# guohaoqiang/Flex

Measured on AMD Instinct MI355X. Metric: SpMM GFLOPS (2*nnz*k/t), higher is better.
Workload: dtype f32

## Files before the change

### flex_amd/csrc/spmm_bf16_kernels.hip

```cpp
#include <cstdint>

#include "attention_device.h"
#include "plan.h"
#include "spmm_device.h"

namespace flex {
namespace spmm_bf16 {

using namespace spmm_dev;
using attention::bf16_bits;

struct Acc8 {
    float4 lo, hi;
};

__device__ __forceinline__ void fma8(Acc8 &acc, float v, const float4 &w) {
    const uint32_t w0 = __float_as_uint(w.x), w1 = __float_as_uint(w.y), w2 = __float_as_uint(w.z), w3 = __float_as_uint(w.w);
    acc.lo.x = fmaf(v, as_f32(w0 << 16), acc.lo.x);
    acc.lo.y = fmaf(v, as_f32(w0 & 0xFFFF0000u), acc.lo.y);
    acc.lo.z = fmaf(v, as_f32(w1 << 16), acc.lo.z);
    acc.lo.w = fmaf(v, as_f32(w1 & 0xFFFF0000u), acc.lo.w);
    acc.hi.x = fmaf(v, as_f32(w2 << 16), acc.hi.x);
    acc.hi.y = fmaf(v, as_f32(w2 & 0xFFFF0000u), acc.hi.y);
    acc.hi.z = fmaf(v, as_f32(w3 << 16), acc.hi.z);
    acc.hi.w = fmaf(v, as_f32(w3 & 0xFFFF0000u), acc.hi.w);
}

__device__ __forceinline__ v4u narrow8(const float4 &lo, const float4 &hi) {
    const v4u r = {bf16_bits(lo.x) | (bf16_bits(lo.y) << 16), bf16_bits(lo.z) | (bf16_bits(lo.w) << 16),
                   bf16_bits(hi.x) | (bf16_bits(hi.y) << 16), bf16_bits(hi.z) | (bf16_bits(hi.w) << 16)};
    return r;
}

template <int G, bool OFF32, int U>
__device__ __forceinline__ void compute_chunk_bf16(const PlanView &p, const ChunkRegs &d, uint2 *my_lds, const char *__restrict__ Bb,
                                                   uint32_t *__restrict__ Cw, int lane, int c0, bool col_ok, uint32_t tile) {
    constexpr int S = 64 / G;
    const int slot = lane / G;
    const uint64_t ldc = static_cast<uint64_t>(p.ldc);
    const uint32_t lane_off = (col_ok ? c0 : c0 - (lane % G) * 4) * 4u;
    const uint64_t row_bytes = static_cast<uint64_t>(p.ldb) * 4u;
    const uint4 hdr = d.hdr;
    const uint2 cx = d.cx;
    const uint32_t my_beg = d.my_beg, my_dst = d.my_dst;

    const uint32_t nt = hdr.y, zb = hdr.z, ze = hdr.w;
    const bool packed_chunk = p.rec_packed != 0 && (cx.y & kChunkWide) == 0;
    const uint2 *__restrict__ rec = p.rec_packed != 0 ? p.rec + cx.x - zb : p.rec;
    uint32_t carry = 0;

    uint32_t ti = 0;
    uint32_t row_end = __builtin_amdgcn_readlane(my_beg, 1);
    Acc8 acc = {{0.f, 0.f, 0.f, 0.f}, {0.f, 0.f, 0.f, 0.f}};
    const bool out_ok = col_ok && slot == 0;
    auto flush = [&](uint32_t pos) {
        do {
            const uint32_t dst = __builtin_amdgcn_readlane(my_dst, ti);
            if ((dst & (kPartialFlag | kBundleFlag)) == (kPartialFlag | kBundleFlag)) {
                if constexpr (kTileHasBundles<G>) {
                    const uint32_t first = dst & (kBundleRowsPerChunk - 1u);
                    const uint32_t held = first < 64u ? d.my_bd0 : d.my_bd1;
                    const uint32_t row = static_cast<uint32_t>(
                        __builtin_amdgcn_ds_bpermute(static_cast<int>(((first & 63u) + slot) << 2), static_cast<int>(held)));
                    if (col_ok && row != kBundleNoRow) {
                        const bool none = (row & kBundleZero) != 0;
                        const v4u zero = {0u, 0u, 0u, 0u};
                        const v4u val = none ? zero : narrow8(acc.lo, acc.hi);
                        __builtin_nontemporal_store(val, reinterpret_cast<v4u *>(Cw + static_cast<uint64_t>(row & ~kBundleZero) * ldc + c0));
                    }
                }
            } else if (__builtin_expect((dst & kPartialFlag) != 0, 0)) {
                const float4 lo = reduce_full<G>(acc.lo), hi = reduce_full<G>(acc.hi);
                if (out_ok) {
                    int l = lane;
                    asm volatile("" : "+v"(l));
                    const int col = 2 * (static_cast<int>(tile) * (4 * G) + (l % G) * 4);
                    float *prow = p.partial + static_cast<uint64_t>(dst & ~kPartialFlag) * (2u * static_cast<uint32_t>(p.k)) + col;
                    *reinterpret_cast<float4 *>(prow) = lo;
                    *reinterpret_cast<float4 *>(prow + 4) = hi;
                }
            } else {
                const float4 lo = reduce_full<G>(acc.lo), hi = reduce_full<G>(acc.hi);
                if (out_ok) __builtin_nontemporal_store(narrow8(lo, hi), reinterpret_cast<v4u *>(Cw + static_cast<uint64_t>(dst) * ldc + c0));
            }
            acc = {{0.f, 0.f, 0.f, 0.f}, {0.f, 0.f, 0.f, 0.f}};
            ++ti;
            row_end = ti < nt ? __builtin_amdgcn_readlane(my_beg, ti + 1) : 0xFFFFFFFFu;
        } while (row_end == pos);
    };
    if (nt == 0) row_end = 0xFFFFFFFFu;
    if (row_end == zb) flush(zb);

    uint32_t pos = zb;
    for (uint32_t wz = zb; wz < ze; wz += kWindowRecs<G>) {
        const uint32_t wn = min(static_cast<uint32_t>(kWindowRecs<G>), ze - wz);
        if (packed_chunk) carry = stage_window_packed<G, OFF32>(p, my_lds, zb, wz, wn, cx, hdr.x, nt, my_beg, carry, static_cast<uint32_t>(row_bytes), lane);
        else stage_window<G>(my_lds, rec, wz, wn, lane, p.rec_nt != 0);
        const uint32_t nsteps = wn / S;
        const uint2 *lds_slot = my_lds + slot;
        uint32_t j = 0;
        for (; j + U <= nsteps; j += U) {
            uint2 r[U];
            float4 b[U];
#pragma unroll
            for (int u = 0; u < U; ++u) r[u] = lds_slot[(j + u) * S];
#pragma unroll
            for (int u = 0; u < U; ++u) b[u] = gather4<OFF32>(Bb, r[u].x, lane_off, row_bytes);
#pragma unroll
            for (int u = 0; u < U; ++u) {
                fma8(acc, as_f32(r[u].y), b[u]);
                pos += S;
                if (pos == row_end) flush(pos);
            }
        }
        if (j < nsteps) {
            uint2 r[U];
            float4 b[U];
#pragma unroll
            for (int u = 0; u < U; ++u) r[u] = lds_slot[min(j + u, nsteps - 1) * S];
#pragma unroll
            for (int u = 0; u < U; ++u) b[u] = gather4<OFF32>(Bb, r[u].x, lane_off, row_bytes);
#pragma unroll
            for (int u = 0; u < U; ++u) {
                if (j + u < nsteps) {
                    fma8(acc, as_f32(r[u].y), b[u]);
                    pos += S;
                    if (pos == row_end) flush(pos);
                }
            }
        }
    }
}

template <int G, bool OFF32>
constexpr int kWavesHint = G == 64 && OFF32 ? 6 : G >= 32 ? 5 : 7;

template <int G, bool OFF32, int U, int WPB>
__global__ __launch_bounds__(64 * WPB) __attribute__((amdgpu_waves_per_eu(kWavesHint<G, OFF32>))) void spmm_flat_bf16_kernel(PlanView p, const flex_bf16 *__restrict__ B,
                                                                                                                  flex_bf16 *__restrict__ C) {
    __shared__ uint2 lds_rec[WPB][kWindowRecs<G>];
    const int lane = threadIdx.x & 63;
    const uint32_t wib = __builtin_amdgcn_readfirstlane(threadIdx.x >> 6);
    uint32_t tile, ktiles, chunk;
    if (!place_of_wave<G, WPB>(p, wib, tile, ktiles, chunk)) return;
    const int c0 = tile * (4 * G) + (lane % G) * 4;
    const bool col_ok = c0 < p.k;
    ChunkRegs d;
    if (!load_chunk<G>(p, chunk, lane, d)) return;
    compute_chunk_bf16<G, OFF32, U>(p, d, lds_rec[wib], reinterpret_cast<const char *>(B), reinterpret_cast<uint32_t *>(C), lane, c0, col_ok, tile);
}

__global__ __launch_bounds__(256) void spmm_fixup_bf16_kernel(const float *__restrict__ partial, const SplitRow *__restrict__ rows, uint32_t n_rows,
                                                              int k, int ldcw, uint32_t *__restrict__ Cw) {
    const int lane = threadIdx.x & 63;
    const uint32_t wib = __builtin_amdgcn_readfirstlane(threadIdx.x >> 6);
    const uint32_t i = blockIdx.x * kWavesPerBlock + wib;
    if (i >= n_rows) return;
    const SplitRow sr = rows[i];
    for (int c = lane; c < k / 2; c += 64) {
        const float *p = partial + static_cast<uint64_t>(sr.first) * k + 2 * c;
        float2 s = make_float2(0.f, 0.f);
        uint32_t j = 0;
        for (; j + 8 <= sr.count; j += 8) {
            float2 v[8];
#pragma unroll
            for (int u = 0; u < 8; ++u) v[u] = *reinterpret_cast<const float2 *>(p + static_cast<uint64_t>(j + u) * k);
#pragma unroll
            for (int u = 0; u < 8; ++u) {
                s.x += v[u].x;
                s.y += v[u].y;
            }
        }
        float2 v[8];
#pragma unroll
        for (int u = 0; u < 8; ++u) v[u] = (j + u < sr.count) ? *reinterpret_cast<const float2 *>(p + static_cast<uint64_t>(j + u) * k) : make_float2(0.f, 0.f);
#pragma unroll
        for (int u = 0; u < 8; ++u)
            if (j + u < sr.count) {
                s.x += v[u].x;
                s.y += v[u].y;
            }
        Cw[static_cast<uint64_t>(sr.row) * ldcw + c] = bf16_bits(s.x) | (bf16_bits(s.y) << 16);
    }
}

template <int G, bool OFF32, int U>
int launch_flat(const PlanView &v, const flex_bf16 *dB, flex_bf16 *dC, hipStream_t s) {
    uint32_t nblk = (v.n_chunks + kWavesPerBlock - 1) / kWavesPerBlock;
    nblk = (nblk + kXcds - 1) / kXcds * kXcds;
    const uint32_t ktiles = (v.k + 4 * G - 1) / (4 * G);
    const dim3 grid = v.tile_group ? dim3(nblk * ktiles, 1) : dim3(nblk, ktiles);
    hipLaunchKernelGGL((spmm_flat_bf16_kernel<G, OFF32, U, kWavesPerBlock>), grid, dim3(64 * kWavesPerBlock), v.lds_extra, s, v, dB, dC);
    FLEX_HIP_TRY(hipGetLastError());
    return FLEX_OK;
}

template <int G, int U>
int launch_flat_off(const PlanView &v, bool off32, const flex_bf16 *dB, flex_bf16 *dC, hipStream_t s) {
    return off32 ? launch_flat<G, true, U>(v, dB, dC, s) : launch_flat<G, false, U>(v, dB, dC, s);
}

int launch(const PlanView &v, int lanes_per_nz, bool off32, const flex_bf16 *dB, flex_bf16 *dC, hipStream_t s) {
    if (v.n_chunks == 0) return FLEX_OK;
    switch (lanes_per_nz) {
        case 4: return launch_flat_off<4, 4>(v, off32, dB, dC, s);
        case 8: return launch_flat_off<8, 4>(v, off32, dB, dC, s);
        case 16: return launch_flat_off<16, 4>(v, off32, dB, dC, s);
        case 32: return launch_flat_off<32, 8>(v, off32, dB, dC, s);
        case 64: return launch_flat_off<64, 8>(v, off32, dB, dC, s);
        default: return FLEX_ERR_UNSUPPORTED;
    }
}

int launch_fixup(const flex_plan *p, flex_bf16 *dC, hipStream_t s) {
    if (p->n_split == 0) return FLEX_OK;
    const uint32_t nblk = (p->n_split + kWavesPerBlock - 1) / kWavesPerBlock;
    hipLaunchKernelGGL(spmm_fixup_bf16_kernel, dim3(nblk), dim3(256), 0, s, p->d_partial.get(), p->d_split.get(), p->n_split, 2 * p->k, p->ldc,
                       reinterpret_cast<uint32_t *>(dC));
    FLEX_HIP_TRY(hipGetLastError());
    return FLEX_OK;
}

}
}

using namespace flex;

extern "C" int flex_spmm_bf16(flex_plan *p, const flex_bf16 *dB, flex_bf16 *dC, flex_stream_t stream) {
    if (!p || !p->bf16) return FLEX_ERR_INVALID;
    if (p->m == 0) return FLEX_OK;
    if (!dC || (!dB && p->nnz > 0)) return FLEX_ERR_INVALID;
    if ((reinterpret_cast<uintptr_t>(dB) | reinterpret_cast<uintptr_t>(dC)) % 16 != 0) return FLEX_ERR_UNSUPPORTED;
    const DeviceScope on(p->device);
    FLEX_HIP_TRY(on.error());
    hipStream_t s = reinterpret_cast<hipStream_t>(stream);
    const LaunchGuard guard(p, s);
    if (guard.begin() != FLEX_OK) return FLEX_ERR_INVALID;
    int rc = spmm_bf16::launch(plan_view(p, false, nullptr), p->lanes_per_nz, p->off32, dB, dC, s);
    if (rc == FLEX_OK) rc = spmm_bf16::launch_fixup(p, dC, s);
    if (rc == FLEX_OK) guard.done();
    return rc;
}
```

### flex_amd/csrc/spmm_device.h

```cpp
#pragma once
#include "internal.h"

namespace flex {
namespace spmm_dev {
__device__ __forceinline__ float as_f32(uint32_t u) { return __uint_as_float(u); }

template <bool OFF32>
__device__ __forceinline__ float4 gather4(const char *__restrict__ Bb, uint32_t recx, uint32_t lane_off,
                                          uint64_t row_bytes) {
    if constexpr (OFF32) {
        return *reinterpret_cast<const float4 *>(Bb + static_cast<uint32_t>(recx + lane_off));
    } else {
        return *reinterpret_cast<const float4 *>(Bb + (static_cast<uint64_t>(recx) * row_bytes + lane_off));
    }
}

__device__ __forceinline__ void fma4(float4 &acc, float v, const float4 &b) {
    acc.x = fmaf(v, b.x, acc.x);
    acc.y = fmaf(v, b.y, acc.y);
    acc.z = fmaf(v, b.z, acc.z);
    acc.w = fmaf(v, b.w, acc.w);
}

typedef float v4f __attribute__((ext_vector_type(4)));
typedef uint32_t v4u __attribute__((ext_vector_type(4)));

__device__ __forceinline__ float pair8(float a, float b) {
    float r;
    asm("s_nop 1\n\t"
        "v_add_f32_dpp %0, %1, %1 row_ror:8 row_mask:0xf bank_mask:0x3\n\t"
        "v_add_f32_dpp %0, %2, %2 row_ror:8 row_mask:0xf bank_mask:0xc"
        : "=&v"(r)
        : "v"(a), "v"(b));
    return r;
}

__device__ __forceinline__ float pair4(float a, float b) {
    float r;
    asm("s_nop 1\n\t"
        "v_add_f32_dpp %0, %1, %1 row_ror:12 row_mask:0xf bank_mask:0x5\n\t"
        "v_add_f32_dpp %0, %2, %2 row_ror:4 row_mask:0xf bank_mask:0xa"
        : "=&v"(r)
        : "v"(a), "v"(b));
    return r;
}

__device__ __forceinline__ float pair16(float a, float b) {
    const auto sw = __builtin_amdgcn_permlane16_swap(__float_as_uint(a), __float_as_uint(b), false, false);
    return __uint_as_float(sw[0]) + __uint_as_float(sw[1]);
}

__device__ __forceinline__ float pair32(float a, float b) {
    const auto sw = __builtin_amdgcn_permlane32_swap(__float_as_uint(a), __float_as_uint(b), false, false);
    return __uint_as_float(sw[0]) + __uint_as_float(sw[1]);
}

template <int G>
__device__ __forceinline__ float4 reduce_full(const float4 &acc) {
    float4 r = acc;
    if constexpr (G <= 4) {
        auto partner = [](float x) {
            const int lo = __builtin_amdgcn_update_dpp(0, __builtin_bit_cast(int, x), 0x12C, 0xf, 0x5, false);
            return __builtin_bit_cast(float, __builtin_amdgcn_update_dpp(lo, __builtin_bit_cast(int, x), 0x124, 0xf, 0xa, false));
        };
        r.x += partner(r.x);
        r.y += partner(r.y);
        r.z += partner(r.z);
        r.w += partner(r.w);
    }
    if constexpr (G <= 8) {
        r.x += __builtin_bit_cast(float, __builtin_amdgcn_update_dpp(0, __builtin_bit_cast(int, r.x), 0x128, 0xf, 0xf, false));
        r.y += __builtin_bit_cast(float, __builtin_amdgcn_update_dpp(0, __builtin_bit_cast(int, r.y), 0x128, 0xf, 0xf, false));
        r.z += __builtin_bit_cast(float, __builtin_amdgcn_update_dpp(0, __builtin_bit_cast(int, r.z), 0x128, 0xf, 0xf, false));
        r.w += __builtin_bit_cast(float, __builtin_amdgcn_update_dpp(0, __builtin_bit_cast(int, r.w), 0x128, 0xf, 0xf, false));
    }
    if constexpr (G <= 16) {
        r.x = pair16(r.x, r.x);
        r.y = pair16(r.y, r.y);
        r.z = pair16(r.z, r.z);
        r.w = pair16(r.w, r.w);
    }
    if constexpr (G <= 32) {
        r.x = pair32(r.x, r.x);
        r.y = pair32(r.y, r.y);
        r.z = pair32(r.z, r.z);
        r.w = pair32(r.w, r.w);
    }
    return r;
}

template <int G>
constexpr int kWindowRecs = G <= 8 ? 512 : 256;
template <int G>
constexpr bool kTileHasBundles = 64 / G >= static_cast<int>(kBundleMinSlots);


typedef uint32_t v2u __attribute__((ext_vector_type(2)));
template <bool NT>
__device__ __forceinline__ uint2 load_rec(const uint2 *ptr) {
    if constexpr (NT) {
        const v2u v = __builtin_nontemporal_load(reinterpret_cast<const v2u *>(ptr));
        return make_uint2(v.x, v.y);
    } else {
        return *ptr;
    }
}

template <bool NT, int LOADS>
__device__ __forceinline__ void stage_n(uint2 *my_lds, const uint2 *__restrict__ rec, uint32_t wz, uint32_t wn, int lane) {
    uint2 r[LOADS];
#pragma unroll
    for (int i = 0; i < LOADS; ++i) r[i] = load_rec<NT>(rec + wz + min(static_cast<uint32_t>(i * 64 + lane), wn - 1));
#pragma unroll
    for (int i = 0; i < LOADS; ++i) my_lds[i * 64 + lane] = r[i];
}

template <bool NT, int G>
__device__ __forceinline__ void stage_window_t(uint2 *my_lds, const uint2 *__restrict__ rec, uint32_t wz, uint32_t wn, int lane) {
    if (wn <= 64) {
        stage_n<NT, 1>(my_lds, rec, wz, wn, lane);
    } else if constexpr (kWindowRecs<G> > 256) {
        if (wn <= 256) stage_n<NT, 4>(my_lds, rec, wz, wn, lane);
        else stage_n<NT, kWindowRecs<G> / 64>(my_lds, rec, wz, wn, lane);
    } else {
        stage_n<NT, 4>(my_lds, rec, wz, wn, lane);
    }
}

template <int G>
__device__ __forceinline__ void stage_window(uint2 *my_lds, const uint2 *__restrict__ rec, uint32_t wz, uint32_t wn, int lane, bool nt) {
    if (nt) stage_window_t<true, G>(my_lds, rec, wz, wn, lane);
    else stage_window_t<false, G>(my_lds, rec, wz, wn, lane);
}

template <bool NT, class T>
__device__ __forceinline__ T load_stream(const T *ptr) {
    if constexpr (NT) return __builtin_nontemporal_load(ptr);
    else return *ptr;
}

template <bool NT, bool PAIR, int LOADS, int R>
__device__ __forceinline__ void stage_packed_n(uint2 *my_lds, const float *__restrict__ val, const uint16_t *__restrict__ dcol, uint32_t wn, int lane,
                                               uint32_t (&vv)[R]) {
    const char *const vb = reinterpret_cast<const char *>(val), *const db = reinterpret_cast<const char *>(dcol);
#pragma unroll
    for (int i = 0; i < R; ++i) vv[i] = 0u;
    if constexpr (PAIR) {
        uint32_t d[LOADS];
#pragma unroll
        for (int i = 0; i < LOADS; ++i) {
            const uint32_t off = min(static_cast<uint32_t>(i * 64 + lane), wn / 2 - 1) * 4u;
            const v2u v = load_stream<NT>(reinterpret_cast<const v2u *>(vb + static_cast<uint32_t>(off * 2u)));
            vv[2 * i] = v.x;
            vv[2 * i + 1] = v.y;
            d[i] = load_stream<NT>(reinterpret_cast<const uint32_t *>(db + off));
        }
#pragma unroll
        for (int i = 0; i < LOADS; ++i) *reinterpret_cast<uint4 *>(my_lds + 2 * (i * 64 + lane)) = make_uint4(d[i] & 0xFFFFu, 0u, d[i] >> 16, 0u);
    } else {
        uint16_t d[LOADS];
#pragma unroll
        for (int i = 0; i < LOADS; ++i) {
            const uint32_t off = min(static_cast<uint32_t>(i * 64 + lane), wn - 1) * 2u;
            vv[i] = __float_as_uint(load_stream<NT>(reinterpret_cast<const float *>(vb + static_cast<uint32_t>(off * 2u))));
            d[i] = load_stream<NT>(reinterpret_cast<const uint16_t *>(db + off));
        }
#pragma unroll
        for (int i = 0; i < LOADS; ++i) my_lds[i * 64 + lane] = make_uint2(d[i], 0u);
    }
}

template <bool NT, int G, int R>
__device__ __forceinline__ void stage_packed_t(uint2 *my_lds, const float *__restrict__ val, const uint16_t *__restrict__ dcol, uint32_t wn, int lane,
                                               uint32_t (&vv)[R]) {
    constexpr bool PAIR = 64 / G >= 2;
    constexpr int PER = PAIR ? 128 : 64, FULL = kWindowRecs<G> / PER;
    if (wn <= PER) stage_packed_n<NT, PAIR, 1>(my_lds, val, dcol, wn, lane, vv);
    else if (FULL > 2 && wn <= 2 * PER) stage_packed_n<NT, PAIR, 2>(my_lds, val, dcol, wn, lane, vv);
    else stage_packed_n<NT, PAIR, FULL>(my_lds, val, dcol, wn, lane, vv);
}

template <int G, bool OFF32>
__device__ __forceinline__ uint32_t stage_window_packed(const PlanView &p, uint2 *my_lds, uint32_t zb, uint32_t wz, uint32_t wn, uint2 cx,
                                                        uint32_t t0, uint32_t nt, uint32_t my_beg, uint32_t carry, uint32_t row_bytes32, int lane) {
    constexpr int W = kWindowRecs<G>, R = W / 64;
    constexpr bool PAIR = 64 / G >= 2;
    asm volatile("" : "+v"(lane));
    uint32_t vv[R];
    if (p.rec_nt != 0) stage_packed_t<true, G>(my_lds, p.rec_val + wz, p.rec_dcol + wz, wn, lane, vv);
    else stage_packed_t<false, G>(my_lds, p.rec_val + wz, p.rec_dcol + wz, wn, lane, vv);
    for (uint32_t j = lane; j < cx.y; j += 64) {
        const uint2 e = p.exc[cx.x + j];
        const uint32_t at = zb + e.x - wz;
        if (at < wn) my_lds[at].x += e.y;
    }
    if (lane == 0) my_lds[0].x += carry;
    const uint32_t next_beg = __shfl_down(my_beg, 1);
    const uint32_t at = my_beg - wz;
    if (static_cast<uint32_t>(lane) < nt && next_beg != my_beg && at < wn) my_lds[at] = make_uint2(p.t_col0[t0 + lane], 1u);
    __builtin_amdgcn_wave_barrier();
    uint32_t w[R], fbits = 0;
#pragma unroll
    for (int i = 0; i < R; ++i) {
        const uint2 s = my_lds[lane * R + i];
        w[i] = s.x;
        fbits |= s.y << i;
    }
    fbits &= (1u << R) - 1u;
    __builtin_amdgcn_wave_barrier();
#pragma unroll
    for (int i = 0; i < R; ++i) my_lds[PAIR ? 2 * ((i / 2) * 64 + lane) + (i & 1) : i * 64 + lane].y = vv[i];
    uint32_t run = 0;
#pragma unroll
    for (int i = 0; i < R; ++i) {
        run = ((fbits >> i) & 1u) ? w[i] : run + w[i];
        w[i] = run;
    }
    uint32_t inc = run;
#pragma unroll
    for (int dlt = 1; dlt < 64; dlt <<= 1) {
        const uint32_t up = __shfl_up(inc, dlt);
        if (lane >= dlt) inc += up;
    }
    const uint32_t exc_sum = inc - run;
    const uint64_t below = __builtin_amdgcn_ballot_w64(fbits != 0) & ((uint64_t(1) << lane) - 1u);
    const int q = below ? 63 - __builtin_clzll(below) : 0;
    const uint32_t e_q = __shfl(exc_sum, q);
    const uint32_t enter = below ? exc_sum - e_q : exc_sum;
    uint32_t last = 0;
#pragma unroll
    for (int i = 0; i < R; ++i) {
        const bool open = (fbits & ((2u << i) - 1u)) == 0;
        const uint32_t col = w[i] + (open ? enter : 0u);
        my_lds[lane * R + i].x = OFF32 ? col * row_bytes32 : col;
        last = col;
    }
    __builtin_amdgcn_wave_barrier();
    return __builtin_amdgcn_readlane(last, 63);
}

template <int G, int WPB>
__device__ __forceinline__ bool place_of_wave(const PlanView &p, uint32_t wib, uint32_t &tile, uint32_t &ktiles, uint32_t &chunk) {
    uint32_t bid;
    tile = blockIdx.y;
    ktiles = gridDim.y;
    if (p.tile_group == 0) {
        const uint32_t cpx = gridDim.x / kXcds;
        bid = p.xcd_remap ? (blockIdx.x % kXcds) * cpx + (blockIdx.x / kXcds) : blockIdx.x;
    } else {
        ktiles = (p.k + 4 * G - 1) / (4 * G);
        const uint32_t nwg = gridDim.x / ktiles;
        const uint32_t slice = p.xcd_remap ? nwg / kXcds : nwg;
        const uint32_t l = p.xcd_remap ? blockIdx.x / kXcds : blockIdx.x;
        const uint32_t g = l / (p.tile_group * ktiles), r = l % (p.tile_group * ktiles);
        const uint32_t g0 = g * p.tile_group, gs = min(p.tile_group, slice - g0);
        tile = r / gs;
        const uint32_t in_slice = g0 + r % gs;
        if (tile >= ktiles) return false;
        bid = p.xcd_remap ? (blockIdx.x % kXcds) * slice + in_slice : in_slice;
    }
    chunk = bid * WPB + wib;
    return chunk < p.n_chunks;
}

struct ChunkRegs {
    uint4 hdr;
    uint2 cx;
    uint32_t my_beg, my_dst;
    uint2 my_aux;
    uint32_t my_bd0, my_bd1;
};

template <int G>
__device__ __forceinline__ bool load_chunk(const PlanView &p, uint32_t chunk, int lane, ChunkRegs &d) {
    const uint4 hdr = d.hdr = p.chunk[chunk];
    uint2 cb = make_uint2(0u, 0u);
    if constexpr (kTileHasBundles<G>)
        if (p.bd_rows != nullptr) cb = p.chunk_bd[chunk];
    uint2 cx = make_uint2(0u, 0u);
    if (p.rec_packed != 0) cx = p.chunk_exc[chunk];
    d.cx = cx;
    if (hdr.y == 0) return false;
    d.my_beg = (static_cast<uint32_t>(lane) <= hdr.y) ? p.t_beg[hdr.x + lane] : 0u;
    d.my_dst = (static_cast<uint32_t>(lane) < hdr.y) ? p.t_dst[hdr.x + lane] : 0u;
    d.my_aux = (static_cast<uint32_t>(lane) < hdr.y) ? p.t_aux[hdr.x + lane] : make_uint2(0u, 0u);
    d.my_bd0 = d.my_bd1 = kBundleNoRow;
    if (kTileHasBundles<G> && cb.y != 0) {
        if (static_cast<uint32_t>(lane) < cb.y) d.my_bd0 = p.bd_rows[cb.x + lane];
        if (static_cast<uint32_t>(lane) + 64u < cb.y) d.my_bd1 = p.bd_rows[cb.x + 64u + lane];
    }
    return true;
}

}
}
```

### flex_amd/csrc/spmm_kernels.hip

```cpp
#include "spmm_device.h"

namespace flex {
namespace {

using namespace spmm_dev;

template <int G>
struct RowOut {
    static constexpr int kVals = G <= 8 ? 1 : 4;
    float v[kVals];
};

template <int G>
__device__ __forceinline__ int row_out_col(int lane, int c0) {
    if constexpr (G == 8) return c0 + 2 * ((lane >> 3) & 1) + ((lane >> 4) & 1);
    else if constexpr (G == 4) return c0 + 2 * ((lane >> 2) & 1) + ((lane >> 3) & 1);
    else return c0;
}

template <int G>
__device__ __forceinline__ bool row_out_lane(int lane) {
    return G == 8 ? lane < 32 : G == 4 ? lane < 16 : lane < G;
}

template <int G>
__device__ __forceinline__ RowOut<G> reduce_row(const float4 &acc) {
    RowOut<G> o;
    if constexpr (G == 8) {
        const float t = pair16(pair8(acc.x, acc.z), pair8(acc.y, acc.w));
        o.v[0] = pair32(t, t);
    } else if constexpr (G == 4) {
        const float t = pair8(pair4(acc.x, acc.z), pair4(acc.y, acc.w));
        const float h = pair16(t, t);
        o.v[0] = pair32(h, h);
    } else {
        float4 r = acc;
        if constexpr (G <= 16) {
            r.x = pair16(r.x, r.x);
            r.y = pair16(r.y, r.y);
            r.z = pair16(r.z, r.z);
            r.w = pair16(r.w, r.w);
        }
        if constexpr (G <= 32) {
            r.x = pair32(r.x, r.x);
            r.y = pair32(r.y, r.y);
            r.z = pair32(r.z, r.z);
            r.w = pair32(r.w, r.w);
        }
        o.v[0] = r.x; o.v[1] = r.y; o.v[2] = r.z; o.v[3] = r.w;
    }
    return o;
}

template <int G>
__device__ __forceinline__ void store_row_out(float *ptr, const RowOut<G> &o) {
    if constexpr (RowOut<G>::kVals == 4) {
        const v4f val = {o.v[0], o.v[1], o.v[2], o.v[3]};
        __builtin_nontemporal_store(val, reinterpret_cast<v4f *>(ptr));
    } else {
        __builtin_nontemporal_store(o.v[0], ptr);
    }
}

__device__ __forceinline__ v4f load_b128_sc1(const float *ptr) {
    v4f v;
    asm volatile("global_load_dwordx4 %0, %1, off sc1" : "=v"(v) : "v"(ptr) : "memory");
    return v;
}

template <int N>
__device__ __forceinline__ void wait_loads(v4f (&v)[N]) {
    static_assert(N == 8, "one batch of the piece sum");
    asm volatile("s_waitcnt vmcnt(0)"
                 : "+v"(v[0]), "+v"(v[1]), "+v"(v[2]), "+v"(v[3]), "+v"(v[4]), "+v"(v[5]), "+v"(v[6]), "+v"(v[7])
                 :
                 : "memory");
}

[[maybe_unused]] __device__ __forceinline__ uint32_t xcc_id() {
    uint32_t x;
    asm volatile("s_getreg_b32 %0, hwreg(HW_REG_XCC_ID)" : "=s"(x));
    return x & (kXcds - 1);
}


template <int G, bool OFF32, int U>
__device__ __forceinline__ void compute_chunk(const PlanView &p, uint4 hdr, uint32_t my_beg, uint32_t my_dst, uint2 my_aux,
                                              uint32_t my_bd0, uint32_t my_bd1, uint2 cx, uint2 *my_lds, const char *__restrict__ Bb,
                                              float *__restrict__ C, int lane, int c0, bool col_ok, uint32_t tile, uint32_t ktiles) {
    constexpr int S = 64 / G;
    const int slot = lane / G;
    const int k = p.k;
    const uint64_t ldc = static_cast<uint64_t>(p.ldc);
    const uint32_t lane_off = (col_ok ? c0 : c0 - (lane % G) * 4) * 4u;
    const uint64_t row_bytes = static_cast<uint64_t>(p.ldb) * 4u;

    const uint32_t nt = hdr.y, zb = hdr.z, ze = hdr.w;
    const bool packed_chunk = p.rec_packed != 0 && (cx.y & kChunkWide) == 0;
    const uint2 *__restrict__ rec = p.rec_packed != 0 ? p.rec + cx.x - zb : p.rec;
    uint32_t carry = 0;

    uint32_t ti = 0;
    uint32_t row_end = __builtin_amdgcn_readlane(my_beg, 1);
    float4 acc = {0.f, 0.f, 0.f, 0.f};
    const int out_col = row_out_col<G>(lane, c0);
    const bool out_ok = col_ok && row_out_lane<G>(lane);
    auto flush = [&](uint32_t pos) {
        do {
            const uint32_t dst = __builtin_amdgcn_readlane(my_dst, ti);
            if ((dst & (kPartialFlag | kBundleFlag)) == (kPartialFlag | kBundleFlag)) {
                if constexpr (kTileHasBundles<G>) {
                    const uint32_t first = dst & (kBundleRowsPerChunk - 1u);
                    const uint32_t held = first < 64u ? my_bd0 : my_bd1;
                    const uint32_t row = static_cast<uint32_t>(
                        __builtin_amdgcn_ds_bpermute(static_cast<int>(((first & 63u) + slot) << 2), static_cast<int>(held)));
                    if (col_ok && row != kBundleNoRow) {
                        const bool none = (row & kBundleZero) != 0;
                        const v4f val = {none ? 0.f : acc.x, none ? 0.f : acc.y, none ? 0.f : acc.z, none ? 0.f : acc.w};
                        __builtin_nontemporal_store(val, reinterpret_cast<v4f *>(C + static_cast<uint64_t>(row & ~kBundleZero) * ldc + c0));
                    }
                }
            } else if (__builtin_expect((dst & kPartialFlag) != 0, 0)) {
                const float4 r = reduce_full<G>(acc);
                float *prow = p.partial + static_cast<uint64_t>(dst & ~kPartialFlag) * k;
                if (slot == 0 && col_ok) {
                    int l = lane;
                    asm volatile("" : "+v"(l));
                    const int col = static_cast<int>(tile) * (4 * G) + (l % G) * 4;
                    if (p.fused_fixup) {
                        const auto prsrc = __builtin_amdgcn_make_buffer_rsrc(prow, 0, k * 4, 0x00020000);
                        const v4u pv = {__float_as_uint(r.x), __float_as_uint(r.y), __float_as_uint(r.z), __float_as_uint(r.w)};
                        __builtin_amdgcn_raw_buffer_store_b128(pv, prsrc, col * 4, 0, 16 );
                    } else {
                        *reinterpret_cast<float4 *>(prow + col) = r;
                    }
                }
            } else {
                const RowOut<G> o = reduce_row<G>(acc);
                if (out_ok) store_row_out<G>(C + static_cast<uint64_t>(dst) * ldc + out_col, o);
            }
            acc = {0.f, 0.f, 0.f, 0.f};
            ++ti;
            row_end = ti < nt ? __builtin_amdgcn_readlane(my_beg, ti + 1) : 0xFFFFFFFFu;
        } while (row_end == pos);
    };
    if (nt == 0) row_end = 0xFFFFFFFFu;
    if (row_end == zb) flush(zb);

    uint32_t pos = zb;
    for (uint32_t wz = zb; wz < ze; wz += kWindowRecs<G>) {
        const uint32_t wn = min(static_cast<uint32_t>(kWindowRecs<G>), ze - wz);
        if (packed_chunk) carry = stage_window_packed<G, OFF32>(p, my_lds, zb, wz, wn, cx, hdr.x, nt, my_beg, carry, static_cast<uint32_t>(row_bytes), lane);
        else stage_window<G>(my_lds, rec, wz, wn, lane, p.rec_nt != 0);
        const uint32_t nsteps = wn / S;
        const uint2 *lds_slot = my_lds + slot;
        uint32_t j = 0;
        for (; j + U <= nsteps; j += U) {
            uint2 r[U];
            float4 b[U];
#pragma unroll
            for (int u = 0; u < U; ++u) r[u] = lds_slot[(j + u) * S];
#pragma unroll
            for (int u = 0; u < U; ++u) b[u] = gather4<OFF32>(Bb, r[u].x, lane_off, row_bytes);
#pragma unroll
            for (int u = 0; u < U; ++u) {
                fma4(acc, as_f32(r[u].y), b[u]);
                pos += S;
                if (pos == row_end) flush(pos);
            }
        }
        if (j < nsteps) {
            uint2 r[U];
            float4 b[U];
#pragma unroll
            for (int u = 0; u < U; ++u) r[u] = lds_slot[min(j + u, nsteps - 1) * S];
#pragma unroll
            for (int u = 0; u < U; ++u) b[u] = gather4<OFF32>(Bb, r[u].x, lane_off, row_bytes);
#pragma unroll
            for (int u = 0; u < U; ++u) {
                if (j + u < nsteps) {
                    fma4(acc, as_f32(r[u].y), b[u]);
                    pos += S;
                    if (pos == row_end) flush(pos);
                }
            }
        }
    }
    const bool mine_partial = static_cast<uint32_t>(lane) < nt && (my_dst & (kPartialFlag | kBundleFlag)) == kPartialFlag;
    if (p.fused_fixup && __builtin_amdgcn_ballot_w64(mine_partial) != 0) {
        asm volatile("s_waitcnt vmcnt(0)" ::: "memory");
        uint32_t arrived = 0;
        if (mine_partial)
            arrived = __hip_atomic_fetch_add(p.split_cnt + static_cast<uint64_t>(my_aux.x) * ktiles + tile, 1u,
                                             __ATOMIC_RELAXED, __HIP_MEMORY_SCOPE_AGENT);
        uint64_t done = __builtin_amdgcn_ballot_w64(mine_partial && arrived + 1 == my_aux.y);
        while (done != 0) {
            int take = -1;
#pragma unroll
            for (int s2 = 0; s2 < S; ++s2) {
                if (done != 0) {
                    const int i = __builtin_ctzll(done);
                    done &= done - 1;
                    if (slot == s2) take = i;
                }
            }
            const uint32_t sidx = __shfl(my_aux.x, take < 0 ? 0 : take);
            if (take >= 0) {
                const SplitRow sr = p.split[sidx];
                if (col_ok) {
                    int l = lane;
                    asm volatile("" : "+v"(l));
                    const int c0 = static_cast<int>(tile) * (4 * G) + (l % G) * 4;
                    const float *base = p.partial + static_cast<uint64_t>(sr.first) * k + c0;
                    float4 s4 = {0.f, 0.f, 0.f, 0.f};
                    for (uint32_t j = 0; j < sr.count; j += 8) {
                        v4f v[8];
#pragma unroll
                        for (int u = 0; u < 8; ++u) v[u] = load_b128_sc1(base + static_cast<uint64_t>(min(j + u, sr.count - 1)) * k);
                        wait_loads(v);
#pragma unroll
                        for (int u = 0; u < 8; ++u) {
                            if (j + u < sr.count) {
                                s4.x += v[u].x;
                                s4.y += v[u].y;
                                s4.z += v[u].z;
                                s4.w += v[u].w;
                            }
                        }
                    }
                    const v4f val = {s4.x, s4.y, s4.z, s4.w};
                    __builtin_nontemporal_store(val, reinterpret_cast<v4f *>(C + static_cast<uint64_t>(sr.row) * ldc + c0));
                }
                if (lane % G == 0)
                    __hip_atomic_store(p.split_cnt + static_cast<uint64_t>(sidx) * ktiles + tile, 0u, __ATOMIC_RELAXED,
                                       __HIP_MEMORY_SCOPE_AGENT);
            }
        }
    }
}

template <int G, bool OFF32, int U, int WPB, bool STAMP = false>
__global__ __launch_bounds__(64 * WPB) __attribute__((amdgpu_waves_per_eu(U == (G >= 32 ? 8 : 4) ? (G >= 32 ? (OFF32 ? 7 : 6) : G >= 16 ? 7 : 8) : 4))) void spmm_flat_kernel(PlanView p, const float *__restrict__ B,
                                                             float *__restrict__ C) {
    __shared__ uint2 lds_rec[WPB][kWindowRecs<G>];
    const int lane = threadIdx.x & 63;
    const uint32_t wib = __builtin_amdgcn_readfirstlane(threadIdx.x >> 6);
    uint32_t tile = blockIdx.y, ktiles = gridDim.y, bid;
    if (p.tile_group == 0) {
        const uint32_t cpx = gridDim.x / kXcds;
        bid = p.xcd_remap ? (blockIdx.x % kXcds) * cpx + (blockIdx.x / kXcds) : blockIdx.x;
    } else {
        ktiles = (p.k + 4 * G - 1) / (4 * G);
        const uint32_t nwg = gridDim.x / ktiles;
        const uint32_t slice = p.xcd_remap ? nwg / kXcds : nwg;
        const uint32_t l = p.xcd_remap ? blockIdx.x / kXcds : blockIdx.x;
        const uint32_t g = l / (p.tile_group * ktiles), r = l % (p.tile_group * ktiles);
        const uint32_t g0 = g * p.tile_group, gs = min(p.tile_group, slice - g0);
        tile = r / gs;
        const uint32_t in_slice = g0 + r % gs;
        if (tile >= ktiles) return;
        bid = p.xcd_remap ? (blockIdx.x % kXcds) * slice + in_slice : in_slice;
    }
    const uint32_t chunk = bid * WPB + wib;
    if (chunk >= p.n_chunks) return;
    const int c0 = tile * (4 * G) + (lane % G) * 4;
    const bool col_ok = c0 < p.k;
    const uint4 hdr = p.chunk[chunk];
    uint2 cb = make_uint2(0u, 0u);
    if constexpr (kTileHasBundles<G>)
        if (p.bd_rows != nullptr) cb = p.chunk_bd[chunk];
    uint2 cx = make_uint2(0u, 0u);
    if (p.rec_packed != 0) cx = p.chunk_exc[chunk];
    if (hdr.y == 0) return;
    const uint32_t my_beg = (static_cast<uint32_t>(lane) <= hdr.y) ? p.t_beg[hdr.x + lane] : 0u;
    const uint32_t my_dst = (static_cast<uint32_t>(lane) < hdr.y) ? p.t_dst[hdr.x + lane] : 0u;
    const uint2 my_aux = (static_cast<uint32_t>(lane) < hdr.y) ? p.t_aux[hdr.x + lane] : make_uint2(0u, 0u);
    uint32_t my_bd0 = kBundleNoRow, my_bd1 = kBundleNoRow;
    if (kTileHasBundles<G> && cb.y != 0) {
        if (static_cast<uint32_t>(lane) < cb.y) my_bd0 = p.bd_rows[cb.x + lane];
        if (static_cast<uint32_t>(lane) + 64u < cb.y) my_bd1 = p.bd_rows[cb.x + 64u + lane];
    }
    uint64_t stamp_t0 = 0;
    if constexpr (STAMP) stamp_t0 = __builtin_amdgcn_s_memrealtime();
    compute_chunk<G, OFF32, U>(p, hdr, my_beg, my_dst, my_aux, my_bd0, my_bd1, cx, lds_rec[wib], reinterpret_cast<const char *>(B), C, lane, c0, col_ok, tile, ktiles);
    if constexpr (STAMP) {
        asm volatile("s_waitcnt vmcnt(0) lgkmcnt(0)" ::: "memory");
        const uint64_t stamp_t1 = __builtin_amdgcn_s_memrealtime();
        if (lane == 0 && p.trace != nullptr) {
            uint32_t hw_id;
            asm volatile("s_getreg_b32 %0, hwreg(HW_REG_HW_ID)" : "=s"(hw_id));
            uint64_t *log = p.trace + (static_cast<uint64_t>(tile) * p.n_chunks + chunk) * 3;
            log[0] = stamp_t0;
            log[1] = stamp_t1;
            log[2] = (static_cast<uint64_t>(xcc_id()) << 32) | hw_id;
        }
    }
}

template <bool OFF32>
__global__ __launch_bounds__(256) void spmm_generic_kernel(PlanView p, const float *__restrict__ B,
                                                           float *__restrict__ C, uint32_t slots_per_step) {
    const int lane = threadIdx.x & 63;
    const uint32_t wib = __builtin_amdgcn_readfirstlane(threadIdx.x >> 6);
    const uint32_t cpx = gridDim.x / kXcds;
    const uint32_t bid = p.xcd_remap ? (blockIdx.x % kXcds) * cpx + (blockIdx.x / kXcds) : blockIdx.x;
    const uint32_t w = bid * kWavesPerBlock + wib;
    if (w >= p.n_chunks) return;
    const int k = p.k;
    const int cb = blockIdx.y * 256 + lane;
    const uint32_t t0 = p.chunk[w].x, t1 = t0 + p.chunk[w].y;
    uint2 cx = make_uint2(0u, 0u);
    if (p.rec_packed != 0 && t1 > t0) cx = p.chunk_exc[w];
    const bool packed_chunk = p.rec_packed != 0 && (cx.y & kChunkWide) == 0;
    const uint32_t cz = p.chunk[w].z;
    const uint2 *__restrict__ rec = p.rec_packed != 0 ? p.rec + cx.x - cz : p.rec;
    uint32_t ei = 0;
    for (uint32_t t = t0; t < t1; ++t) {
        const uint32_t zb = p.t_beg[t], ze = p.t_beg[t + 1];
        const uint32_t dst = p.t_dst[t];
        if ((dst & (kPartialFlag | kBundleFlag)) == (kPartialFlag | kBundleFlag)) {
            const uint2 a = p.t_aux[t];
            const uint32_t slots = slots_per_step;
            for (uint32_t s = 0; s < slots; ++s) {
                const uint32_t row = p.bd_rows[a.x + s];
                if (row == kBundleNoRow) continue;
                float acc[4] = {0.f, 0.f, 0.f, 0.f};
                if ((row & kBundleZero) == 0) {
                    for (uint32_t j = 0; j < a.y; ++j) {
                        const uint2 r = rec[zb + j * slots + s];
                        const float v = as_f32(r.y);
                        const float *brow = OFF32 ? reinterpret_cast<const float *>(reinterpret_cast<const char *>(B) + r.x)
                                                  : B + static_cast<uint64_t>(r.x) * p.ldb;
#pragma unroll
                        for (int i = 0; i < 4; ++i) {
                            const int c = cb + 64 * i;
                            if (c < k) acc[i] = fmaf(v, brow[c], acc[i]);
                        }
                    }
                }
                float *orow = C + static_cast<uint64_t>(row & ~kBundleZero) * p.ldc;
#pragma unroll
                for (int i = 0; i < 4; ++i) {
                    const int c = cb + 64 * i;
                    if (c < k) orow[c] = acc[i];
                }
            }
            continue;
        }
        float acc[4] = {0.f, 0.f, 0.f, 0.f};
        uint32_t col = packed_chunk ? p.t_col0[t] : 0u;
        for (uint32_t z = zb; z < ze; ++z) {
            uint2 r;
            if (packed_chunk) {
                uint32_t d = p.rec_dcol[z];
                if (ei < cx.y && p.exc[cx.x + ei].x == z - cz) d += p.exc[cx.x + ei++].y;
                col += d;
                r = make_uint2(OFF32 ? col * (static_cast<uint32_t>(p.ldb) * 4u) : col, __float_as_uint(p.rec_val[z]));
            } else {
                r = rec[z];
            }
            const float v = as_f32(r.y);
            const float *brow = OFF32 ? reinterpret_cast<const float *>(reinterpret_cast<const char *>(B) + r.x)
                                      : B + static_cast<uint64_t>(r.x) * p.ldb;
#pragma unroll
            for (int i = 0; i < 4; ++i) {
                const int c = cb + 64 * i;
                if (c < k) acc[i] = fmaf(v, brow[c], acc[i]);
            }
        }
        float *orow = (dst & kPartialFlag) ? p.partial + static_cast<uint64_t>(dst & ~kPartialFlag) * k
                                           : C + static_cast<uint64_t>(dst) * p.ldc;
#pragma unroll
        for (int i = 0; i < 4; ++i) {
            const int c = cb + 64 * i;
            if (c < k) orow[c] = acc[i];
        }
    }
}

__global__ __launch_bounds__(256) void spmm_fixup_kernel(const float *__restrict__ partial,
                                                         const SplitRow *__restrict__ rows, uint32_t n_rows,
                                                         int k, int ldc, float *__restrict__ C) {
    const int lane = threadIdx.x & 63;
    const uint32_t wib = __builtin_amdgcn_readfirstlane(threadIdx.x >> 6);
    const uint32_t i = blockIdx.x * kWavesPerBlock + wib;
    if (i >= n_rows) return;
    const SplitRow sr = rows[i];
    for (int c = lane; c < k; c += 64) {
        const float *p = partial + static_cast<uint64_t>(sr.first) * k + c;
        float s = 0.f;
        uint32_t j = 0;
        for (; j + 8 <= sr.count; j += 8) {
            float v[8];
#pragma unroll
            for (int u = 0; u < 8; ++u) v[u] = p[static_cast<uint64_t>(j + u) * k];
#pragma unroll
            for (int u = 0; u < 8; ++u) s += v[u];
        }
        float v[8];
#pragma unroll
        for (int u = 0; u < 8; ++u) v[u] = (j + u < sr.count) ? p[static_cast<uint64_t>(j + u) * k] : 0.f;
#pragma unroll
        for (int u = 0; u < 8; ++u)
            if (j + u < sr.count) s += v[u];
        C[static_cast<uint64_t>(sr.row) * ldc + c] = s;
    }
}

template <bool VEC4>
__global__ __launch_bounds__(256) void gather_rows_kernel(float *__restrict__ dst, const float *__restrict__ src,
                                                          const int32_t *__restrict__ idx, int64_t n, int k) {
    const int lane = threadIdx.x & 63;
    const int64_t nwaves = static_cast<int64_t>(gridDim.x) * kWavesPerBlock;
    for (int64_t r = static_cast<int64_t>(blockIdx.x) * kWavesPerBlock + (threadIdx.x >> 6); r < n; r += nwaves) {
        const int64_t s = idx[r];
        if constexpr (VEC4) {
            const float4 *sp = reinterpret_cast<const float4 *>(src + s * k);
            float4 *dp = reinterpret_cast<float4 *>(dst + r * k);
            for (int c = lane; c < k / 4; c += 64) dp[c] = sp[c];
        } else {
            for (int c = lane; c < k; c += 64) dst[r * k + c] = src[s * k + c];
        }
    }
}

template <int G, bool OFF32, int U>
int launch_v4(const PlanView &v, const float *dB, float *dC, hipStream_t s) {
    uint32_t nblk = (v.n_chunks + kWavesPerBlock - 1) / kWavesPerBlock;
    nblk = (nblk + kXcds - 1) / kXcds * kXcds;
    const uint32_t ktiles = (v.k + 4 * G - 1) / (4 * G);
    const dim3 grid = v.tile_group ? dim3(nblk * ktiles, 1) : dim3(nblk, ktiles);
    hipLaunchKernelGGL((spmm_flat_kernel<G, OFF32, U, kWavesPerBlock>), grid, dim3(64 * kWavesPerBlock), v.lds_extra, s, v, dB, dC);
    FLEX_HIP_TRY(hipGetLastError());
    return FLEX_OK;
}

template <int G, int U>
int launch_stamped(const PlanView &v, bool off32, const float *dB, float *dC, hipStream_t s) {
    uint32_t nblk = (v.n_chunks + kWavesPerBlock - 1) / kWavesPerBlock;
    nblk = (nblk + kXcds - 1) / kXcds * kXcds;
    const uint32_t ktiles = (v.k + 4 * G - 1) / (4 * G);
    const dim3 grid = v.tile_group ? dim3(nblk * ktiles, 1) : dim3(nblk, ktiles);
    if (off32)
        hipLaunchKernelGGL((spmm_flat_kernel<G, true, U, kWavesPerBlock, true>), grid, dim3(64 * kWavesPerBlock), v.lds_extra, s, v, dB, dC);
    else
        hipLaunchKernelGGL((spmm_flat_kernel<G, false, U, kWavesPerBlock, true>), grid, dim3(64 * kWavesPerBlock), v.lds_extra, s, v, dB, dC);
    FLEX_HIP_TRY(hipGetLastError());
    return FLEX_OK;
}

template <int G, int U>
int launch_v4_off(const PlanView &v, bool off32, const float *dB, float *dC, hipStream_t s) {
    return off32 ? launch_v4<G, true, U>(v, dB, dC, s) : launch_v4<G, false, U>(v, dB, dC, s);
}

}

int launch_spmm(const PlanView &v, int lanes_per_nz, bool off32, bool vec4, const float *dB, float *dC,
                hipStream_t s, int unroll) {
    if (v.n_chunks == 0) return FLEX_OK;
    if (!vec4) {
        uint32_t nblk = (v.n_chunks + kWavesPerBlock - 1) / kWavesPerBlock;
        nblk = (nblk + kXcds - 1) / kXcds * kXcds;
        const uint32_t ktiles = (v.k + 255) / 256;
        if (off32)
            hipLaunchKernelGGL((spmm_generic_kernel<true>), dim3(nblk, ktiles), dim3(256), 0, s, v, dB, dC, 64u / static_cast<uint32_t>(lanes_per_nz));
        else
            hipLaunchKernelGGL((spmm_generic_kernel<false>), dim3(nblk, ktiles), dim3(256), 0, s, v, dB, dC, 64u / static_cast<uint32_t>(lanes_per_nz));
        FLEX_HIP_TRY(hipGetLastError());
        return FLEX_OK;
    }
    if (unroll == 8) {
        switch (lanes_per_nz) {
            case 8: return launch_v4_off<8, 8>(v, off32, dB, dC, s);
            case 16: return launch_v4_off<16, 8>(v, off32, dB, dC, s);
            default: break;
        }
    }
    switch (lanes_per_nz) {
        case 4: return launch_v4_off<4, 4>(v, off32, dB, dC, s);
        case 8: return launch_v4_off<8, 4>(v, off32, dB, dC, s);
        case 16: return launch_v4_off<16, 4>(v, off32, dB, dC, s);
        case 32: return launch_v4_off<32, 8>(v, off32, dB, dC, s);
        case 64: return launch_v4_off<64, 8>(v, off32, dB, dC, s);
        default: return FLEX_ERR_UNSUPPORTED;
    }
}

int launch_spmm_stamped(const PlanView &v, int lanes_per_nz, bool off32, const float *dB, float *dC, hipStream_t s) {
    if (v.n_chunks == 0) return FLEX_OK;
    switch (lanes_per_nz) {
        case 4: return launch_stamped<4, 4>(v, off32, dB, dC, s);
        case 8: return launch_stamped<8, 4>(v, off32, dB, dC, s);
        case 16: return launch_stamped<16, 4>(v, off32, dB, dC, s);
        case 32: return launch_stamped<32, 8>(v, off32, dB, dC, s);
        case 64: return launch_stamped<64, 8>(v, off32, dB, dC, s);
        default: return FLEX_ERR_UNSUPPORTED;
    }
}

int kernel_attributes(int lanes_per_nz, bool off32, bool vec4, hipFuncAttributes *attr, int *waves_per_cu) {
    const void *fn = nullptr;
    if (!vec4) {
        fn = off32 ? reinterpret_cast<const void *>(spmm_generic_kernel<true>) : reinterpret_cast<const void *>(spmm_generic_kernel<false>);
    } else {
        switch (lanes_per_nz) {
            case 4: fn = off32 ? reinterpret_cast<const void *>(spmm_flat_kernel<4, true, 4, kWavesPerBlock>) : reinterpret_cast<const void *>(spmm_flat_kernel<4, false, 4, kWavesPerBlock>); break;
            case 8: fn = off32 ? reinterpret_cast<const void *>(spmm_flat_kernel<8, true, 4, kWavesPerBlock>) : reinterpret_cast<const void *>(spmm_flat_kernel<8, false, 4, kWavesPerBlock>); break;
            case 16: fn = off32 ? reinterpret_cast<const void *>(spmm_flat_kernel<16, true, 4, kWavesPerBlock>) : reinterpret_cast<const void *>(spmm_flat_kernel<16, false, 4, kWavesPerBlock>); break;
            case 32: fn = off32 ? reinterpret_cast<const void *>(spmm_flat_kernel<32, true, 8, kWavesPerBlock>) : reinterpret_cast<const void *>(spmm_flat_kernel<32, false, 8, kWavesPerBlock>); break;
            case 64: fn = off32 ? reinterpret_cast<const void *>(spmm_flat_kernel<64, true, 8, kWavesPerBlock>) : reinterpret_cast<const void *>(spmm_flat_kernel<64, false, 8, kWavesPerBlock>); break;
            default: return FLEX_ERR_UNSUPPORTED;
        }
    }
    FLEX_HIP_TRY(hipFuncGetAttributes(attr, fn));
    int blocks = 0;
    FLEX_HIP_TRY(hipOccupancyMaxActiveBlocksPerMultiprocessor(&blocks, fn, 64 * kWavesPerBlock, 0));
    *waves_per_cu = blocks * kWavesPerBlock;
    return FLEX_OK;
}

int launch_fixup(const float *partial, const SplitRow *rows, uint32_t n_rows, int k, int ldc, float *dC, hipStream_t s) {
    if (n_rows == 0) return FLEX_OK;
    const uint32_t nblk = (n_rows + kWavesPerBlock - 1) / kWavesPerBlock;
    hipLaunchKernelGGL(spmm_fixup_kernel, dim3(nblk), dim3(256), 0, s, partial, rows, n_rows, k, ldc, dC);
    FLEX_HIP_TRY(hipGetLastError());
    return FLEX_OK;
}

int launch_gather_rows(float *dst, const float *src, const int32_t *idx, int64_t n, int k, hipStream_t s) {
    if (n <= 0) return FLEX_OK;
    const int64_t want = (n + kWavesPerBlock - 1) / kWavesPerBlock;
    const uint32_t nblk = static_cast<uint32_t>(want < 2048 ? want : 2048);
    const bool vec4 = (k % 4 == 0) && ((reinterpret_cast<uintptr_t>(dst) | reinterpret_cast<uintptr_t>(src)) % 16 == 0);
    if (vec4)
        hipLaunchKernelGGL((gather_rows_kernel<true>), dim3(nblk), dim3(256), 0, s, dst, src, idx, n, k);
    else
        hipLaunchKernelGGL((gather_rows_kernel<false>), dim3(nblk), dim3(256), 0, s, dst, src, idx, n, k);
    FLEX_HIP_TRY(hipGetLastError());
    return FLEX_OK;
}

}
```

Before: 8602.

## Issue first window record loads early and use DPP prefix scan

For small group sizes (G<=8), the first window's packed record loads, column-start and exception loads are split out and issued before the row-end setup and initial flush, so their latency overlaps that setup. The window loop is restructured so later windows are staged after the compute of the current one. The 64-lane shuffle-based inclusive scan is replaced with DPP row_shr and row_bcast operations. Asm marker comments are also added to the staging routines. This adds register pressure from holding the first window's values across the prologue.

```diff
diff --git a/flex_amd/csrc/spmm_bf16_kernels.hip b/flex_amd/csrc/spmm_bf16_kernels.hip
--- a/flex_amd/csrc/spmm_bf16_kernels.hip
+++ b/flex_amd/csrc/spmm_bf16_kernels.hip
@@ -48,6 +48,13 @@
     const bool packed_chunk = p.rec_packed != 0 && (cx.y & kChunkWide) == 0;
     const uint2 *__restrict__ rec = p.rec_packed != 0 ? p.rec + cx.x - zb : p.rec;
     uint32_t carry = 0;
+
+    uint32_t wn = min(static_cast<uint32_t>(kWindowRecs<G>), ze - zb);
+    WindowRegs<G> first;
+    if (kFirstWindowEarly<G> && wn != 0) {
+        if (packed_chunk) issue_window_packed<G>(p, my_lds, zb, wn, cx, hdr.x, nt, lane, first);
+        else stage_window<G>(my_lds, rec, zb, wn, lane, p.rec_nt != 0);
+    }
 
     uint32_t ti = 0;
     uint32_t row_end = __builtin_amdgcn_readlane(my_beg, 1);
@@ -92,10 +99,13 @@
     if (row_end == zb) flush(zb);
 
     uint32_t pos = zb;
-    for (uint32_t wz = zb; wz < ze; wz += kWindowRecs<G>) {
-        const uint32_t wn = min(static_cast<uint32_t>(kWindowRecs<G>), ze - wz);
-        if (packed_chunk) carry = stage_window_packed<G, OFF32>(p, my_lds, zb, wz, wn, cx, hdr.x, nt, my_beg, carry, static_cast<uint32_t>(row_bytes), lane);
-        else stage_window<G>(my_lds, rec, wz, wn, lane, p.rec_nt != 0);
+    if constexpr (kFirstWindowEarly<G>) {
+        if (wn != 0 && packed_chunk) carry = finish_window_packed<G, OFF32>(p, my_lds, zb, zb, wn, cx, nt, my_beg, 0u, static_cast<uint32_t>(row_bytes), lane, first);
+    } else if (wn != 0) {
+        if (packed_chunk) carry = stage_window_packed<G, OFF32>(p, my_lds, zb, zb, wn, cx, hdr.x, nt, my_beg, 0u, static_cast<uint32_t>(row_bytes), lane);
+        else stage_window<G>(my_lds, rec, zb, wn, lane, p.rec_nt != 0);
+    }
+    for (uint32_t wz = zb; wz < ze;) {
         const uint32_t nsteps = wn / S;
         const uint2 *lds_slot = my_lds + slot;
         uint32_t j = 0;
@@ -128,6 +138,12 @@
                     if (pos == row_end) flush(pos);
                 }
             }
+        }
+        wz += kWindowRecs<G>;
+        if (wz < ze) {
+            wn = min(static_cast<uint32_t>(kWindowRecs<G>), ze - wz);
+            if (packed_chunk) carry = stage_window_packed<G, OFF32>(p, my_lds, zb, wz, wn, cx, hdr.x, nt, my_beg, carry, static_cast<uint32_t>(row_bytes), lane);
+            else stage_window<G>(my_lds, rec, wz, wn, lane, p.rec_nt != 0);
         }
     }
 }
diff --git a/flex_amd/csrc/spmm_device.h b/flex_amd/csrc/spmm_device.h
--- a/flex_amd/csrc/spmm_device.h
+++ b/flex_amd/csrc/spmm_device.h
@@ -113,6 +113,7 @@
     for (int i = 0; i < LOADS; ++i) r[i] = load_rec<NT>(rec + wz + min(static_cast<uint32_t>(i * 64 + lane), wn - 1));
 #pragma unroll
     for (int i = 0; i < LOADS; ++i) my_lds[i * 64 + lane] = r[i];
+    asm volatile("; staged, variant %0" ::"n"(LOADS + (NT ? 16 : 0)) : "memory");
 }
 
 template <bool NT, int G>
@@ -168,6 +169,7 @@
 #pragma unroll
         for (int i = 0; i < LOADS; ++i) my_lds[i * 64 + lane] = make_uint2(d[i], 0u);
     }
+    asm volatile("; staged, variant %0" ::"n"(LOADS + (NT ? 16 : 0)) : "memory");
 }
 
 template <bool NT, int G, int R>
@@ -180,16 +182,40 @@
     else stage_packed_n<NT, PAIR, FULL>(my_lds, val, dcol, wn, lane, vv);
 }
 
+template <int G>
+constexpr bool kFirstWindowEarly = G <= 8;
+
+template <int G>
+struct WindowRegs {
+    uint32_t vv[kWindowRecs<G> / 64];
+    uint32_t col0;
+    uint2 exc0;
+};
+
+template <int G>
+__device__ __forceinline__ void issue_window_packed(const PlanView &p, uint2 *my_lds, uint32_t wz, uint32_t wn, uint2 cx, uint32_t t0, uint32_t nt,
+                                                    int lane, WindowRegs<G> &r) {
+    asm volatile("" : "+v"(lane));
+    r.col0 = p.t_col0[t0 + min(static_cast<uint32_t>(lane), max(nt, 1u) - 1u)];
+    r.exc0 = make_uint2(0u, 0u);
+    if (cx.y != 0) r.exc0 = p.exc[cx.x + min(static_cast<uint32_t>(lane), cx.y - 1u)];
+    if (p.rec_nt != 0) stage_packed_t<true, G>(my_lds, p.rec_val + wz, p.rec_dcol + wz, wn, lane, r.vv);
+    else stage_packed_t<false, G>(my_lds, p.rec_val + wz, p.rec_dcol + wz, wn, lane, r.vv);
+}
+
 template <int G, bool OFF32>
-__device__ __forceinline__ uint32_t stage_window_packed(const PlanView &p, uint2 *my_lds, uint32_t zb, uint32_t wz, uint32_t wn, uint2 cx,
-                                                        uint32_t t0, uint32_t nt, uint32_t my_beg, uint32_t carry, uint32_t row_bytes32, int lane) {
+__device__ __forceinline__ uint32_t finish_window_packed(const PlanView &p, uint2 *my_lds, uint32_t zb, uint32_t wz, uint32_t wn, uint2 cx,
+                                                         uint32_t nt, uint32_t my_beg, uint32_t carry, uint32_t row_bytes32, int lane,
+                                                         const WindowRegs<G> &r) {
     constexpr int W = kWindowRecs<G>, R = W / 64;
     constexpr bool PAIR = 64 / G >= 2;
     asm volatile("" : "+v"(lane));
-    uint32_t vv[R];
-    if (p.rec_nt != 0) stage_packed_t<true, G>(my_lds, p.rec_val + wz, p.rec_dcol + wz, wn, lane, vv);
-    else stage_packed_t<false, G>(my_lds, p.rec_val + wz, p.rec_dcol + wz, wn, lane, vv);
-    for (uint32_t j = lane; j < cx.y; j += 64) {
+    const uint32_t(&vv)[R] = r.vv;
+    if (static_cast<uint32_t>(lane) < cx.y) {
+        const uint32_t at = zb + r.exc0.x - wz;
+        if (at < wn) my_lds[at].x += r.exc0.y;
+    }
+    for (uint32_t j = lane + 64u; j < cx.y; j += 64) {
         const uint2 e = p.exc[cx.x + j];
         const uint32_t at = zb + e.x - wz;
         if (at < wn) my_lds[at].x += e.y;
@@ -197,7 +223,7 @@
     if (lane == 0) my_lds[0].x += carry;
     const uint32_t next_beg = __shfl_down(my_beg, 1);
     const uint32_t at = my_beg - wz;
-    if (static_cast<uint32_t>(lane) < nt && next_beg != my_beg && at < wn) my_lds[at] = make_uint2(p.t_col0[t0 + lane], 1u);
+    if (static_cast<uint32_t>(lane) < nt && next_beg != my_beg && at < wn) my_lds[at] = make_uint2(r.col0, 1u);
     __builtin_amdgcn_wave_barrier();
     uint32_t w[R], fbits = 0;
 #pragma unroll
@@ -217,11 +243,12 @@
         w[i] = run;
     }
     uint32_t inc = run;
-#pragma unroll
-    for (int dlt = 1; dlt < 64; dlt <<= 1) {
-        const uint32_t up = __shfl_up(inc, dlt);
-        if (lane >= dlt) inc += up;
-    }
+    inc += static_cast<uint32_t>(__builtin_amdgcn_update_dpp(0, static_cast<int>(inc), 0x111, 0xf, 0xf, true));
+    inc += static_cast<uint32_t>(__builtin_amdgcn_update_dpp(0, static_cast<int>(inc), 0x112, 0xf, 0xf, true));
+    inc += static_cast<uint32_t>(__builtin_amdgcn_update_dpp(0, static_cast<int>(inc), 0x114, 0xf, 0xf, true));
+    inc += static_cast<uint32_t>(__builtin_amdgcn_update_dpp(0, static_cast<int>(inc), 0x118, 0xf, 0xf, true));
+    inc += static_cast<uint32_t>(__builtin_amdgcn_update_dpp(0, static_cast<int>(inc), 0x142, 0xa, 0xf, false));
+    inc += static_cast<uint32_t>(__builtin_amdgcn_update_dpp(0, static_cast<int>(inc), 0x143, 0xc, 0xf, false));
     const uint32_t exc_sum = inc - run;
     const uint64_t below = __builtin_amdgcn_ballot_w64(fbits != 0) & ((uint64_t(1) << lane) - 1u);
     const int q = below ? 63 - __builtin_clzll(below) : 0;
@@ -237,6 +264,14 @@
     }
     __builtin_amdgcn_wave_barrier();
     return __builtin_amdgcn_readlane(last, 63);
+}
+
+template <int G, bool OFF32>
+__device__ __forceinline__ uint32_t stage_window_packed(const PlanView &p, uint2 *my_lds, uint32_t zb, uint32_t wz, uint32_t wn, uint2 cx,
+                                                        uint32_t t0, uint32_t nt, uint32_t my_beg, uint32_t carry, uint32_t row_bytes32, int lane) {
+    WindowRegs<G> r;
+    issue_window_packed<G>(p, my_lds, wz, wn, cx, t0, nt, lane, r);
+    return finish_window_packed<G, OFF32>(p, my_lds, zb, wz, wn, cx, nt, my_beg, carry, row_bytes32, lane, r);
 }
 
 template <int G, int WPB>
diff --git a/flex_amd/csrc/spmm_kernels.hip b/flex_amd/csrc/spmm_kernels.hip
--- a/flex_amd/csrc/spmm_kernels.hip
+++ b/flex_amd/csrc/spmm_kernels.hip
@@ -99,6 +99,13 @@
     const bool packed_chunk = p.rec_packed != 0 && (cx.y & kChunkWide) == 0;
     const uint2 *__restrict__ rec = p.rec_packed != 0 ? p.rec + cx.x - zb : p.rec;
     uint32_t carry = 0;
+
+    uint32_t wn = min(static_cast<uint32_t>(kWindowRecs<G>), ze - zb);
+    WindowRegs<G> first;
+    if (kFirstWindowEarly<G> && wn != 0) {
+        if (packed_chunk) issue_window_packed<G>(p, my_lds, zb, wn, cx, hdr.x, nt, lane, first);
+        else stage_window<G>(my_lds, rec, zb, wn, lane, p.rec_nt != 0);
+    }
 
     uint32_t ti = 0;
     uint32_t row_end = __builtin_amdgcn_readlane(my_beg, 1);
@@ -148,10 +155,13 @@
     if (row_end == zb) flush(zb);
 
     uint32_t pos = zb;
-    for (uint32_t wz = zb; wz < ze; wz += kWindowRecs<G>) {
-        const uint32_t wn = min(static_cast<uint32_t>(kWindowRecs<G>), ze - wz);
-        if (packed_chunk) carry = stage_window_packed<G, OFF32>(p, my_lds, zb, wz, wn, cx, hdr.x, nt, my_beg, carry, static_cast<uint32_t>(row_bytes), lane);
-        else stage_window<G>(my_lds, rec, wz, wn, lane, p.rec_nt != 0);
+    if constexpr (kFirstWindowEarly<G>) {
+        if (wn != 0 && packed_chunk) carry = finish_window_packed<G, OFF32>(p, my_lds, zb, zb, wn, cx, nt, my_beg, 0u, static_cast<uint32_t>(row_bytes), lane, first);
+    } else if (wn != 0) {
+        if (packed_chunk) carry = stage_window_packed<G, OFF32>(p, my_lds, zb, zb, wn, cx, hdr.x, nt, my_beg, 0u, static_cast<uint32_t>(row_bytes), lane);
+        else stage_window<G>(my_lds, rec, zb, wn, lane, p.rec_nt != 0);
+    }
+    for (uint32_t wz = zb; wz < ze;) {
         const uint32_t nsteps = wn / S;
         const uint2 *lds_slot = my_lds + slot;
         uint32_t j = 0;
@@ -184,6 +194,12 @@
                     if (pos == row_end) flush(pos);
                 }
             }
+        }
+        wz += kWindowRecs<G>;
+        if (wz < ze) {
+            wn = min(static_cast<uint32_t>(kWindowRecs<G>), ze - wz);
+            if (packed_chunk) carry = stage_window_packed<G, OFF32>(p, my_lds, zb, wz, wn, cx, hdr.x, nt, my_beg, carry, static_cast<uint32_t>(row_bytes), lane);
+            else stage_window<G>(my_lds, rec, wz, wn, lane, p.rec_nt != 0);
         }
     }
     const bool mine_partial = static_cast<uint32_t>(lane) < nt && (my_dst & (kPartialFlag | kBundleFlag)) == kPartialFlag;
```

Result: no change. 8592, median of 2 (-0.1%).
